# huziqi/NALO-SLAM

Hardware: AMD Instinct MI355X
Metric: keyframes/sec, KITTI-00 dense 8-KF photometric BA; pose RMSE vs ref (higher is better)
Workload: dtype f32; 1 GPU; kitti00_8kf; image=1224x368, levels=4, window_frames=8, active_points=2000, residuals=14000, tracked_frames_per_keyframe=3, multi_gpu=replicas (window too small to shard)

## Files before the change

nalo-slam_amd/csrc/ba_device.h:

```cpp
#pragma once
#include <cstddef>
#include <hip/hip_runtime.h>
#include <cstdint>

namespace nalo {

constexpr int kBlk = 256;
constexpr int kTopVals = 93;
constexpr int kTopStride = 96;
constexpr int kPreStride = 40;
constexpr int kThSmallSlots = 16384;
constexpr int kPreDirectSlots = 32768;
constexpr int kThDblAB = 1024, kThDblC = 256;

enum : uint8_t { RS_STATE_MASK = 3, RS_EXISTS = 4, RS_ACTIVE = 8, RS_LINEARIZED = 16 };
enum : uint8_t { PT_VALID = 1, PT_MARG = 2, PT_HAS_PRIOR = 4, PT_DROP = 8 };
enum : uint8_t { DEC_KEEP = 0, DEC_DROP_NORES = 1, DEC_DROP = 2, DEC_MARGINALIZE = 3 };

struct BADev {
    int W, P, Ppad, nblocks, w, h;
    const float* calib;
    const float4* img[16];
    const float* img_t[16];
    int wt;
    int lin_sub;
    const float* pre;
    float* frameTH;
    const int* blk_host;
    const int* blk_order;
    int xcd_len;
    float4* pt_geo;
    const float4 *pt_col0, *pt_col1, *pt_w0, *pt_w1;
    float* pt_prior;
    uint8_t* pt_flags;
    float4* pt_acc;
    float4* pt_hcd;
    uint8_t* pt_ngood;
    int* pt_numgood; uint32_t* pt_last;
    float* pt_step;
    float* pt_backup;
    const unsigned* gate_p; unsigned* gate_err; unsigned gate_p_want;
    const float* adF;
    float* pt_relbs;
    float* pt_relbs_next;
    uint8_t* rs_state;
    float2* rs_energy;
    float4 *rs_jp0, *rs_jp1;
    float4* rs_pp0; float2* rs_pp1;
    float4* rs_cpt;
    float* en_new;
    double *th_bufAB, *th_bufC;
    unsigned* th_state;
    double* top_partial;
    double* sc_partial;
    int sc_split;
    const int* host_blk;
    const int* sc_grp;
    int sc_bpw, sc_groups;
    int fix_a, fix_b;
    int reset_oob;
    int no_th;
    double* noapply_E;
};

constexpr int kXadArgFrames = 8;
struct XadArg { float v[4 + kXadArgFrames * kXadArgFrames * 8]; };

struct GateBlock { unsigned x_seq, p_seq, err, pad[29]; float x[4 + NALO_MAX_WINDOW * NALO_MAX_WINDOW * 8]; };
static_assert(offsetof(GateBlock, x) == 128, "flags and payload of the gate block on separate cache lines");
constexpr unsigned kGateCancel = 0xFFFFFFFFu;
struct GateArg { const unsigned* flag; unsigned* err; const float* x; unsigned want; };
__device__ __forceinline__ bool gate_wait(const unsigned* flag, unsigned want, unsigned* err) {
    {
        unsigned v0;
        asm volatile("s_load_dword %0, %1, 0x0\n\ts_waitcnt lgkmcnt(0)" : "=s"(v0) : "s"(flag) : "memory");
        if (v0 == want) { __atomic_signal_fence(__ATOMIC_ACQUIRE); return true; }
    }
    for (unsigned spins = 0; spins < (1u << 21); ++spins) {
        const unsigned v = __hip_atomic_load(flag, __ATOMIC_RELAXED, __HIP_MEMORY_SCOPE_SYSTEM);
        if (v == want) { __atomic_signal_fence(__ATOMIC_ACQUIRE); return true; }
        if (v == kGateCancel) return false;
        __builtin_amdgcn_s_sleep(2);
    }
    if (err) __hip_atomic_store(err, 1u, __ATOMIC_RELAXED, __HIP_MEMORY_SCOPE_SYSTEM);
    return false;
}

struct RedExtra {
    const float* th_en; int th_n; float* th_out;
    double* pub; double seq; unsigned* ticket; const float* th_src;
};

struct StitchDev {
    const double* AD;
    const double *M_top, *M_sc;
    double* H;
    unsigned* ticket;
    int W, n1, NPL;
};

struct StitchLayout {
    size_t top, sc, misc, step, th, flag, npub, lo, dev_size, host_size;
    constexpr StitchLayout(int n1, int W)
        : top(0), sc((size_t)n1 * n1), misc(2 * sc), step(misc + 2 * (size_t)W * W), th(step + 3), flag(th + 2), npub(flag),
          lo((npub + 15) & ~(size_t)15), dev_size(lo + kThDblC), host_size(step + 16) {}
};
static_assert(StitchLayout(21, 2).npub - StitchLayout(21, 2).misc == 2 * 2 * 2 + 5 && StitchLayout(21, 2).th - StitchLayout(21, 2).misc == 2 * 2 * 2 + 5 - 2,
              "StitchLayout and ba_reduce_kernel's tail disagree");

struct CarryDev {
    const int* src;
    int trow[16];
    int W_new, Ppad_new, Ppad_old, enter;
    const float4 *o_geo, *o_col0, *o_col1, *o_w0, *o_w1; const float* o_prior; const uint8_t *o_flags, *o_state; const int* o_ng; const uint32_t* o_last;
    float4 *geo, *col0, *col1, *w0, *w1; float* prior; uint8_t *flags, *state; int* ng; uint32_t* last;
    float4 *acc, *hcd; float *step, *backup, *relbs, *relbs2; uint8_t* ngood; float2* energy; float4 *jp0, *jp1, *cpt;
    const float* imm; int immN;
    const int* a_sel; const float* a_idepth; const uint8_t* a_in;
};
void ba_launch_carry(hipStream_t s, const CarryDev& A, int nblocks);

void ba_launch_sc(hipStream_t s, const BADev& B, int T, int shift, float priorScaleMarg, int margOnly);
void ba_launch_linearize(hipStream_t s, const BADev& B, int mode, int fix, hipEvent_t ev_start = nullptr, hipEvent_t ev_stop = nullptr);
void ba_launch_reset_oob(hipStream_t s, const BADev& B);
void ba_launch_restore(hipStream_t s, const BADev& B, const float4* geo, const uint8_t* state, const uint8_t* flags, const float* prior, const float* th);
void ba_launch_reduce(hipStream_t s, const BADev& B, const int* host_blk, int NPL, double* acc13, double* misc, double* G, bool top, bool sc,
                      const float* step_partial, int step_blocks, double* step_out, bool with_th, double* pub, double seq, unsigned* ticket);
void ba_launch_resub_step(hipStream_t s, const BADev& B, float stepfacD, float* partial, const XadArg& karg, bool karg_is_x);
int ba_launch_stitch(hipStream_t s, const StitchDev& D, size_t* lds_allowed, bool top, bool sc, double* mapped, int ntail, double seq);
void ba_launch_resub(hipStream_t s, const BADev& B, const XadArg& karg, bool karg_is_x);
void ba_launch_resub_step_gated(hipStream_t s, const BADev& B, float stepfacD, float* partial, const GateArg& gate);
void ba_launch_pull(hipStream_t s, float* dst, const float* src_mapped, int n);
void ba_launch_step(hipStream_t s, const BADev& B, float stepfacD, float* partial, double* out3);
void ba_launch_step_sums(hipStream_t s, const BADev& B, const float* partial, double* out3);
void ba_launch_publish(hipStream_t s, const double* src, double* dst_mapped, int n, double seq, unsigned* ticket);
void ba_launch_th_install(hipStream_t s, const double* tail2, float* th);
void ba_launch_th_tail(hipStream_t s, const float* th, double* tail2);
void ba_launch_energy_th(hipStream_t s, const BADev& B);
void ba_launch_set_th(hipStream_t s, float* dst, const float* th, int W);
void ba_launch_energy_th_step(hipStream_t s, const BADev& B, int step);
void ba_launch_lenergy(hipStream_t s, const BADev& B, double* partial);
void ba_launch_load_backup(hipStream_t s, const BADev& B);
void ba_launch_swgray(hipStream_t s, const BADev& B, const double* Rt, double* partial);
void ba_launch_set_idepth(hipStream_t s, const BADev& B, int mode, int host_sel, double scale);
void ba_launch_trk_ref_gather(hipStream_t s, const BADev& B, const int* kmap, float* out);
void ba_launch_hist_update(hipStream_t s, const BADev& B, int scrub_only);
void ba_launch_hist_remap(hipStream_t s, const BADev& B, int idx);
void ba_launch_flag_points(hipStream_t s, const BADev& B, unsigned frame_mask, uint8_t* decision, float* idepth_hessian, int* counts, int* counts_next);
void ba_launch_remove_flagged(hipStream_t s, const BADev& B);

}
```

nalo-slam_amd/csrc/host_ba.hip:

```cpp
#include "nalo_internal.h"
#include "ba_device.h"

namespace nalo {

struct HostFrame {
    int slot = 0, frameID = 0;
    SE3 evalPT, PRE_worldToCam, PRE_camToWorld;
    double state[10] = {}, state_zero[10] = {}, state_scaled[10] = {}, step[10] = {}, state_backup[10] = {};
    float ab_exposure = 1.f, frameEnergyTH = 8 * 8 * kPatternNum;
    double prior[8] = {}, delta[8] = {}, delta_prior[8] = {};
    double ns_pose[6][6] = {}, ns_scale[6] = {};
};

struct BAWindow {
    int W = 0, P = 0, Ppad = 0, nblocks = 0, n = 0, n1 = 0, T = 1, NPL = 16;
    double c_value[4] = {}, c_value_zero[4] = {}, c_value_scaled[4] = {}, c_step[4] = {}, c_value_backup[4] = {};
    float c_scaledf[4] = {}, c_scaledi[4] = {};
    std::vector<HostFrame> frames;
    std::vector<double> adHost, adTarget, HM, bM, lastX, Sproj, solve_scratch;
    std::vector<double> ad_key; int ad_key_W = 0;
    std::vector<int> solve_perm;
    std::vector<float> adHostF, adTargetF, adHTdeltaF;
    float cDeltaF[4] = {};
    bool proj_valid = false;
    bool ad_pending = false;
    int resInA = 0, resInL = 0, resInM = 0;
    std::vector<int> d2p, p2d, blk_host_h, host_blk_h;
    std::vector<uint8_t> flags_h;
    BADev dev{};
    DevBuf<float> pre, frameTH, pt_prior, pt_step, pt_backup, pt_relbs, pt_relbs2, en_new, step_partial;
    DevBuf<double> top_partial, sc_partial;
    unsigned long long pub_seq = 0; bool step_pending = false; int last_canbreak = 0; float st_sumA = 0, st_sumB = 0, st_sumT = 0, st_sumR = 0;
    DevBuf<float4> pt_geo, pt_col0, pt_col1, pt_w0, pt_w1, pt_acc, pt_hcd, rs_jp0, rs_jp1, rs_cpt;
    DevBuf<float2> rs_energy, rs_pp1;
    DevBuf<float4> rs_pp0;
    DevBuf<uint8_t> pt_flags, pt_ngood, rs_state;
    DevBuf<int> blk_host, host_blk, blk_order, sc_grp;
    DevBuf<unsigned> th_hist;
    bool step_fused = false, step_sums_deferred = false;
    bool th_pending = false;
    DevBuf<double> acc13, G, AD, stitched;
    StitchLayout lay = StitchLayout(0, 0);
    size_t stitch_lds_allowed = 48 * 1024;
    DevBuf<unsigned> st_ticket;
    StitchDev sd{};
    HostBuf<double> ad_host;
    Event ev_ad;
    HostBuf<double> stitched_host;
    HostBuf<float> up_host;
    HostBuf<float> pre_map[4]; long pre_pos = 0, pre_synced = 0;
    bool have_lin = false, have_sc = false, stitched_top = false, stitched_sc = false, points_set = false, res_set = false;
    bool pt_acc_on_read = false;
    int sc_shift = -1;
    DevBuf<float4> snap_geo; DevBuf<uint8_t> snap_state, snap_flags; DevBuf<float> snap_prior;
    std::vector<HostFrame> snap_frames; std::vector<double> snap_HM, snap_bM; std::vector<uint8_t> snap_flags_h; bool have_snap = false;
    double snap_calib[4] = {}, snap_calib_scaled[4] = {}; float snap_scaledf[4] = {}, snap_scaledi[4] = {};
    HostBuf<GateBlock> gate_h; unsigned gate_x_seq = 0, gate_p_seq = 0;
    bool want_prelaunch = false, resub_pre = false, lin_pre = false;
    nalo_allreduce_fn hook = nullptr;
    void* hook_user = nullptr;
    bool hook_stream_ordered = false;
    nalo_allreduce_fn hook_side = nullptr; void* hook_side_user = nullptr;
    DevBuf<double> th_buf;
    Event ev_lin, ev_th; bool th_side_inflight = false;
    bool th_lo_pending = false;
    bool never_break = false;
    DevBuf<double> small_sum;
    DevBuf<double> noapply_E; std::vector<double> noapply_h;
    int opt_iterations = 0, opt_rejected = 0;
    bool prior_next = false;
    bool prior_carry = false;
    bool lin_fixed = false;
    std::vector<int> ref_kmap_h; DevBuf<int> ref_kmap; bool ref_kmap_ok = false;
    DevBuf<float> ref_in;
    DevBuf<int> pt_numgood, snap_numgood; DevBuf<uint32_t> pt_last, snap_last;
    bool hist_set = false, snap_hist = false;
    DevBuf<uint8_t> flag_dec; DevBuf<float> flag_H; DevBuf<int> flag_counts; int flag_buf = 0;
    bool flagged = false;
    DevBuf<float4> pt_geo2, pt_col0_2, pt_col1_2, pt_w0_2, pt_w1_2; DevBuf<float> pt_prior2; DevBuf<uint8_t> pt_flags2, rs_state2; DevBuf<int> pt_numgood2; DevBuf<uint32_t> pt_last2;
    std::vector<unsigned long long> key_h;
    std::vector<int> row_of;
    bool carry_ok = false;
    unsigned frames_epoch = 0;
    HostBuf<int> carry_host; DevBuf<int> carry_src; Event ev_carry;
    std::vector<int> carry_map_h; int carry_stats[4] = {}; bool carried = false;
};

void ba_destroy(nalo_ctx* c) {
    delete c->ba;
    c->ba = nullptr;
}

static void calib_set_value(BAWindow& w, const double v[4]) {
    for (int i = 0; i < 4; ++i) w.c_value[i] = v[i];
    w.c_value_scaled[0] = kScaleF * v[0]; w.c_value_scaled[1] = kScaleF * v[1]; w.c_value_scaled[2] = kScaleC * v[2]; w.c_value_scaled[3] = kScaleC * v[3];
    for (int i = 0; i < 4; ++i) w.c_scaledf[i] = (float)w.c_value_scaled[i];
    w.c_scaledi[0] = 1.0f / w.c_scaledf[0]; w.c_scaledi[1] = 1.0f / w.c_scaledf[1];
    w.c_scaledi[2] = -w.c_scaledf[2] / w.c_scaledf[0]; w.c_scaledi[3] = -w.c_scaledf[3] / w.c_scaledf[1];
}
static void frame_set_state(HostFrame& f, const double st[10]) {
    std::memcpy(f.state, st, sizeof(f.state));
    for (int i = 0; i < 3; ++i) f.state_scaled[i] = kScaleXiTrans * st[i];
    for (int i = 3; i < 6; ++i) f.state_scaled[i] = kScaleXiRot * st[i];
    f.state_scaled[6] = kScaleA * st[6]; f.state_scaled[7] = kScaleB * st[7]; f.state_scaled[8] = kScaleA * st[8]; f.state_scaled[9] = kScaleB * st[9];
    f.PRE_worldToCam = se3_exp(f.state_scaled) * f.evalPT;
    f.PRE_camToWorld = f.PRE_worldToCam.inverse();
}
static void frame_set_state_zero(HostFrame& f, const double sz[10]) {
    std::memcpy(f.state_zero, sz, sizeof(f.state_zero));
    const SE3 inv = f.evalPT.inverse();
    for (int i = 0; i < 6; ++i) {
        double eps[6] = {0, 0, 0, 0, 0, 0}, lp[6], lm[6];
        eps[i] = 1e-3; const SE3 P = (f.evalPT * se3_exp(eps)) * inv;
        eps[i] = -1e-3; const SE3 M = (f.evalPT * se3_exp(eps)) * inv;
        se3_log(P, lp); se3_log(M, lm);
        for (int r = 0; r < 6; ++r) f.ns_pose[i][r] = (lp[r] - lm[r]) / (2e-3);
    }
    SE3 P = f.evalPT, M = f.evalPT;
    for (int i = 0; i < 3; ++i) { P.m[i * 4 + 3] *= 1.00001; M.m[i * 4 + 3] /= 1.00001; }
    double lp[6], lm[6];
    se3_log(P * inv, lp); se3_log(M * inv, lm);
    for (int r = 0; r < 6; ++r) f.ns_scale[r] = (lp[r] - lm[r]) / (2e-3);
}
static void frame_take_data(const nalo_settings& set, HostFrame& f) {
    double p[8] = {0, 0, 0, 0, 0, 0, 0, 0};
    if (f.frameID == 0) { for (int i = 0; i < 3; ++i) p[i] = kInitialTransPrior; for (int i = 3; i < 6; ++i) p[i] = kInitialRotPrior; p[6] = kInitialAffPrior; p[7] = kInitialAffPrior; }
    else { p[6] = set.affineOptModeA < 0 ? kInitialAffPrior : set.affineOptModeA; p[7] = set.affineOptModeB < 0 ? kInitialAffPrior : set.affineOptModeB; }
    for (int i = 0; i < 8; ++i) { f.prior[i] = p[i]; f.delta[i] = f.state[i] - f.state_zero[i]; f.delta_prior[i] = f.state[i]; }
}

static int upload_adjoints(nalo_ctx* c);
static int set_adjoints(nalo_ctx* c, bool defer = false) {
    BAWindow& w = *c->ba;
    HostTimer ht(c, "ba.set_adjoints");
    const int W = w.W, n1 = w.n1;
    constexpr int KEY = 15;
    std::vector<uint8_t> dirty(W, 1);
    if (w.ad_key_W == W && w.ad_key.size() == (size_t)W * KEY && w.adHost.size() == (size_t)W * W * 64) {
        for (int f = 0; f < W; ++f) {
            double k[KEY]; std::memcpy(k, w.frames[f].evalPT.m, 12 * sizeof(double)); k[12] = w.frames[f].ab_exposure; k[13] = w.frames[f].state_zero[6]; k[14] = w.frames[f].state_zero[7];
// ... 216 lines not shown
        hipStream_t st = on_side ? c->side : c->stream;
        nalo_allreduce_fn fn = (on_side && w.hook_side) ? w.hook_side : w.hook;
        void* user = (on_side && w.hook_side) ? w.hook_side_user : w.hook_user;
        if (on_side) NALO_HIP(c, hipStreamWaitEvent(c->side, lin_done, 0));
        for (int lvl = 0; lvl < 2; ++lvl) {
            ba_launch_energy_th_step(st, w.dev, lvl);
            if (!w.hook_stream_ordered) NALO_HIP(c, hipStreamSynchronize(st));
            { int rh = call_hook(c, fn, user, w.th_buf.p + lvl * kThDblAB, kThDblAB); if (rh) return rh; }
        }
        ba_launch_energy_th_step(st, w.dev, 2);
        if (on_side) { NALO_HIP(c, hipEventRecord(w.ev_th, c->side)); w.th_side_inflight = true; }
        w.th_lo_pending = true;
    } else if (mode == 0) w.th_pending = true;
    if (fix != 2) { w.have_lin = true; w.have_sc = false; w.stitched_top = false; w.stitched_sc = false; }
    NALO_HIP(c, hipGetLastError());
    w.lin_fixed = mode == 0 && fix == 1;
    return NALO_OK;
}
static int linearize_noapply(nalo_ctx* c, double* E) {
    BAWindow& w = *c->ba;
    const size_t n = (size_t)w.nblocks * w.dev.lin_sub * w.W;
    NALO_HIP(c, w.noapply_E.reserve(n));
    w.dev.noapply_E = w.noapply_E.p;
    NALO_HIP(c, hipMemsetAsync(w.noapply_E.p, 0, n * sizeof(double), c->stream));
    int rc = linearize_async(c, 0, 2); if (rc) return rc;
    w.noapply_h.resize(n);
    NALO_HIP(c, hipMemcpyAsync(w.noapply_h.data(), w.noapply_E.p, n * sizeof(double), hipMemcpyDeviceToHost, c->stream));
    NALO_HIP(c, hipStreamSynchronize(c->stream));
    double s = 0; for (double v : w.noapply_h) s += v;
    { int rs = sum_over_ranks(c, &s, 1); if (rs) return rs; }
    *E = s;
    return NALO_OK;
}
static int calc_l_energy(nalo_ctx* c, double* E) {
    BAWindow& w = *c->ba;
    double e = 0;
    for (const auto& f : w.frames) for (int i = 0; i < 8; ++i) e += f.delta_prior[i] * f.prior[i] * f.delta_prior[i];
    { float ec = 0; for (int i = 0; i < 4; ++i) ec += (w.cDeltaF[i] * (float)kInitialCalibHessian) * w.cDeltaF[i]; e += ec; }
    const int nb = (w.Ppad + 255) / 256;
    NALO_HIP(c, w.noapply_E.reserve((size_t)std::max<size_t>(nb, (size_t)w.nblocks * w.dev.lin_sub * w.W)));
    ba_launch_lenergy(c->stream, w.dev, w.noapply_E.p);
    std::vector<double> part(nb);
    NALO_HIP(c, hipMemcpyAsync(part.data(), w.noapply_E.p, nb * sizeof(double), hipMemcpyDeviceToHost, c->stream));
    NALO_HIP(c, hipStreamSynchronize(c->stream));
    double ep = 0; for (double v : part) ep += v;
    { int rs = sum_over_ranks(c, &ep, 1); if (rs) return rs; }
    *E = e + (double)(float)ep;
    return NALO_OK;
}
static double calc_m_energy(const BAWindow& w) {
    const int n = w.n;
    std::vector<double> d(n);
    for (int i = 0; i < 4; ++i) d[i] = (double)w.cDeltaF[i];
    for (int h = 0; h < w.W; ++h) for (int i = 0; i < 8; ++i) d[4 + 8 * h + i] = w.frames[h].delta[i];
    double E = 0;
    for (int i = 0; i < n; ++i) { double s = 0; for (int j = 0; j < n; ++j) s += w.HM[(size_t)i * n + j] * d[j]; E += d[i] * (2 * w.bM[i] + s); }
    return E;
}
static int load_state_backup(nalo_ctx* c) {
    BAWindow& w = *c->ba;
    calib_set_value(w, w.c_value_backup);
    for (auto& f : w.frames) frame_set_state(f, f.state_backup);
    ba_launch_load_backup(c->stream, w.dev);
    NALO_HIP(c, hipGetLastError());
    return set_precalc(c);
}
static int sc_async(nalo_ctx* c, int shift, float margScale, int margOnly) {
    BAWindow& w = *c->ba;
    ProfScope ps(c, "ba_sc");
    ba_launch_sc(c->stream, w.dev, w.T, shift, margScale, margOnly);
    w.have_sc = true; w.sc_shift = shift; w.stitched_sc = false;
    NALO_HIP(c, hipGetLastError());
    return NALO_OK;
}
static bool prelaunch_eligible(const nalo_ctx* c, const BAWindow& w) {
    return !w.hook && c->set.forceAcceptStep && w.points_set && w.Ppad <= kPreDirectSlots && w.W <= 8;
}
static int prelaunch_iteration(nalo_ctx* c) {
    BAWindow& w = *c->ba;
    if (!w.gate_h.p) {
        NALO_HIP(c, w.gate_h.reserve(1, hipHostMallocMapped | hipHostMallocCoherent));
        std::memset(w.gate_h.p, 0, sizeof(GateBlock));
    }
    GateBlock* const gh = w.gate_h.p; GateBlock* const gd = w.gate_h.dev;
    if (w.pre_pos + 1 - 4 > w.pre_synced || !w.pre_map[0].dev) return NALO_OK;
    if (gh->x_seq == kGateCancel) __atomic_store_n(&gh->x_seq, 0u, __ATOMIC_RELEASE);
    if (gh->p_seq == kGateCancel) __atomic_store_n(&gh->p_seq, 0u, __ATOMIC_RELEASE);
    if (++w.gate_x_seq == kGateCancel) w.gate_x_seq = 1;
    if (++w.gate_p_seq == kGateCancel) w.gate_p_seq = 1;
    {
        ProfScope ps(c, "ba_resub");
        NALO_HIP(c, w.step_partial.reserve((size_t)(w.Ppad / 256 + 1) * 4));
        const GateArg g{&gd->x_seq, &gd->err, gd->x, w.gate_x_seq};
        ba_launch_resub_step_gated(c->stream, w.dev, 1.f, w.step_partial.p, g);
    }
    w.resub_pre = true;
    {
        BADev D = w.dev;
        const size_t nfl = (size_t)w.W * w.W * kPreStride;
        D.pre = w.pre_map[(w.pre_pos + 1) & 3].dev; D.calib = D.pre + nfl;
        D.gate_p = &gd->p_seq; D.gate_err = &gd->err; D.gate_p_want = w.gate_p_seq;
        ProfScope ps(c, "ba_linearize", true);
        ba_launch_linearize(c->stream, D, 0, 0, ps.a, ps.b);
    }
    w.lin_pre = true;
    NALO_HIP(c, hipGetLastError());
    return NALO_OK;
}
static void prelaunch_cancel(nalo_ctx* c) {
    BAWindow& w = *c->ba;
    if (!(w.resub_pre || w.lin_pre) || !w.gate_h.p) return;
    __atomic_store_n(&w.gate_h.p->x_seq, kGateCancel, __ATOMIC_RELEASE); __atomic_store_n(&w.gate_h.p->p_seq, kGateCancel, __ATOMIC_RELEASE);
    (void)hipStreamSynchronize(c->stream);
    w.resub_pre = w.lin_pre = false; w.want_prelaunch = false;
    w.have_lin = false; w.have_sc = false;
}

static int stitch_and_fetch(nalo_ctx* c, bool want_top, bool want_sc, bool th_to_host = false, bool misc_only = false) {
    BAWindow& w = *c->ba;
    if (w.ad_pending && !misc_only) { int ra = upload_adjoints(c); if (ra) return ra; }
    const int NPL = w.NPL, W = w.W;
    const StitchLayout& L = w.lay;
    bool did = false;
    const int ntail = (int)(L.npub - L.misc);
    const double seq = (double)(w.pub_seq + 1);
    double* const dmap = w.stitched_host.dev;
    const bool top = want_top && !w.stitched_top, sc = want_sc && !w.stitched_sc;
    const bool sc_was_summed = w.stitched_sc;
    const bool fuse_lo = w.hook && w.th_lo_pending && (top || misc_only);
    bool th_after_publish = false;
    {
        const bool small_th = !w.hook && w.th_pending && th_to_host && w.dev.Ppad <= kThSmallSlots && (top || sc);
        const bool pub_in_reduce = misc_only && !w.hook && (top || sc) && (small_th || !w.th_pending);
        if ((top || sc) && (th_to_host || w.hook) && !fuse_lo && !pub_in_reduce) {
            if (!small_th) { int rc = flush_th(c); if (rc) return rc; }
            if (!small_th) ba_launch_th_tail(c->stream, w.frameTH.p + (W - 1), w.stitched.p + L.th);
        }
        ProfScope ps(c, "ba_reduce");
        if (top || sc) {
            ba_launch_reduce(c->stream, w.dev, w.host_blk.p, NPL, w.acc13.p, w.stitched.p + L.misc, w.G.p, top, sc,
                             w.step_sums_deferred ? w.step_partial.p : nullptr, (w.Ppad + 255) / 256, w.stitched.p + L.step, small_th,
                             pub_in_reduce ? dmap + L.misc : nullptr, seq, w.st_ticket.p + 2);
            if (small_th) w.th_pending = false;
            w.step_sums_deferred = false;
            if (misc_only) { if (!w.hook && !pub_in_reduce) ba_launch_publish(c->stream, w.stitched.p + L.misc, dmap + L.misc, ntail, seq, w.st_ticket.p + 1); }
            else {
                if (small_th && th_to_host) ba_launch_th_tail(c->stream, w.frameTH.p + (W - 1), w.stitched.p + L.th);
                if (ba_launch_stitch(c->stream, w.sd, &w.stitch_lds_allowed, top, sc, w.hook ? nullptr : dmap, ntail, seq)) return fail(c, NALO_ERR_HIP, "ba_stitch_kernel: LDS size rejected");
                if (top) w.stitched_top = true;
                if (sc) w.stitched_sc = true;
            }
            did = true;
        }
    }
    NALO_HIP(c, hipGetLastError());
    if (did) {
        ++w.pub_seq;
        if (w.hook) {
            const size_t off = misc_only ? L.misc : 0;
            const size_t tail_end = fuse_lo ? L.lo + kThDblC : L.npub;
            size_t ra[2], rb[2]; int nr = 0;
            if (misc_only) { ra[nr] = L.misc; rb[nr++] = tail_end; }
            else if (top && (sc || !sc_was_summed)) { ra[nr] = L.top; rb[nr++] = tail_end; }
            else if (top) { ra[nr] = L.top; rb[nr++] = L.sc; ra[nr] = L.misc; rb[nr++] = tail_end; }
            else { ra[nr] = L.sc; rb[nr++] = L.misc; }
            if (fuse_lo) {
                if (w.th_side_inflight) { NALO_HIP(c, hipStreamWaitEvent(c->stream, w.ev_th, 0)); w.th_side_inflight = false; }
                w.th_lo_pending = false;
            }
            if (!w.hook_stream_ordered) NALO_HIP(c, hipStreamSynchronize(c->stream));
            for (int i = 0; i < nr; ++i) { int rh = call_hook(c, w.hook, w.hook_user, w.stitched.p + ra[i], (int)(rb[i] - ra[i])); if (rh) return rh; }
            if (fuse_lo) {
                if (th_to_host) {
                    ba_launch_energy_th_step(c->stream, w.dev, 3);
                    ba_launch_th_tail(c->stream, w.frameTH.p + (W - 1), w.stitched.p + L.th);
                } else th_after_publish = true;
            } else if (top || misc_only) ba_launch_th_install(c->stream, w.stitched.p + L.th, w.frameTH.p + (W - 1));
            ba_launch_publish(c->stream, w.stitched.p + off, dmap + off, (int)(L.npub - off), seq, w.st_ticket.p + 1);
            if (th_after_publish) ba_launch_energy_th_step(c->stream, w.dev, 3);
            NALO_HIP(c, hipGetLastError());
        }
        { int rc = flush_th(c); if (rc) return rc; }
        if (w.want_prelaunch) { w.want_prelaunch = false; int rc = prelaunch_iteration(c); if (rc) return rc; }
        if (!poll_flag(c, &w.stitched_host.p[L.flag], seq)) return NALO_ERR_HIP;
// ... 1402 lines not shown
```

nalo-slam_amd/csrc/kernels_ba.hip:

```cpp
#include "nalo_internal.h"
#include "ba_device.h"
#include "reduce.h"

namespace nalo {


__global__ __launch_bounds__(256) void ba_reset_oob_kernel(uint8_t* __restrict__ rs_state, float2* __restrict__ rs_energy, size_t n) {
    const size_t i = (size_t)blockIdx.x * blockDim.x + threadIdx.x;
    if (i >= n) return;
    const uint8_t st = rs_state[i];
    if ((st & RS_EXISTS) && !(st & RS_LINEARIZED)) { rs_state[i] = (uint8_t)(st & ~RS_STATE_MASK); rs_energy[i] = make_float2(0.f, 0.f); }
}

struct ScPoint { float4 pa; float4 hc; int ngood; };
__device__ __forceinline__ void sc_point_finish(const BADev& B, int d, ScPoint& P, float prior, float idepth, float idepth_zero, int margOnly, float priorScaleMarg, int shiftPriorToZero) {
    B.pt_hcd[d] = P.hc; B.pt_ngood[d] = (uint8_t)P.ngood;
    if (P.ngood == 0) { P.pa.z = 0.f; P.pa.w = 0.f; }
    else {
        if (margOnly) { prior *= priorScaleMarg; B.pt_prior[d] = prior; }
        float Hs = P.pa.x + prior;
        if (Hs < 1e-10f) Hs = 1e-10f;
        P.pa.z = (float)(1.0 / (double)Hs);
        P.pa.w = P.pa.y;
        if (shiftPriorToZero) P.pa.w += prior * (idepth - idepth_zero);
// ... 559 lines not shown
                if (c < 4) { for (int q = 0; q < nb; ++q) s += U[q * 104 + r * 13 + c]; }
                else if (c == n) { for (int q = 0; q < nb; ++q) s += U[q * 104 + r * 13 + 12]; }
                else {
                    const int j = (c - 4) >> 3, cp = (c - 4) & 7;
                    if (j == a) {
                        for (int q = 0; q < nb; ++q)
#pragma unroll
                            for (int k = 0; k < 8; ++k) s += U[q * 104 + r * 13 + 4 + k] * As[q * kAdMat + cp * kAdRow + k];
                    } else {
                        const int jj = j < a ? j : j - 1, q1 = jj, q2 = W - 1 + jj;
#pragma unroll
                        for (int k = 0; k < 8; ++k) s += U[q1 * 104 + r * 13 + 4 + k] * Ao[q1 * kAdMat + cp * kAdRow + k];
#pragma unroll
                        for (int k = 0; k < 8; ++k) s += U[q2 * 104 + r * 13 + 4 + k] * Ao[q2 * kAdMat + cp * kAdRow + k];
                    }
                }
                put(4 + 8 * a + r, c, s);
                if (c < 4 || c == n) put(c, 4 + 8 * a + r, s);
            }
        } else if (sys == 0) {
            for (int e = tid; e < W * W * 25; e += NT) {
                const int bin = e / 25, o = e - bin * 25, ri = o / 5, ci = o - ri * 5;
                lds[e] = (bin % W != bin / W) ? D.M_top[(size_t)bin * 169 + (ri < 4 ? ri : 12) * 13 + (ci < 4 ? ci : 12)] : 0.0;
            }
            __syncthreads();
            for (int e = tid; e < 25; e += NT) {
                const int ri = e / 5, ci = e - ri * 5;
                double s = 0;
                for (int bin = 0; bin < W * W; ++bin) s += lds[bin * 25 + e];
                put(ri < 4 ? ri : n, ci < 4 ? ci : n, s);
            }
        } else if (g < W) {
            if (ad_in_lds) { if (D.W == 8) stitch_sc_rows<true, 8>(D, lds, g, r0, 8 / kScSplit, put); else stitch_sc_rows<true, 0>(D, lds, g, r0, 8 / kScSplit, put); }
            else stitch_sc_rows<false, 0>(D, lds, g, r0, 8 / kScSplit, put);
        } else {
            const int cb = 8 * (W - 1);
            for (int e = tid; e < W * 25; e += NT) {
                const int i = e / 25, o = e - i * 25, ri = o / 5, ci = o - ri * 5;
                lds[e] = D.M_sc[(size_t)i * NPL * NPL + (size_t)(cb + ri) * NPL + cb + ci];
            }
            __syncthreads();
            for (int e = tid; e < 25; e += NT) {
                const int ri = e / 5, ci = e - ri * 5;
                double s = 0;
                for (int i = 0; i < W; ++i) s += lds[i * 25 + e];
                put(ri < 4 ? ri : n, ci < 4 ? ci : n, s);
            }
        }
    }
    if (!mapped) return;
    __builtin_amdgcn_fence(__ATOMIC_RELEASE, "workgroup");
    __syncthreads();
    if (tid == 0) is_last = __hip_atomic_fetch_add(D.ticket, 1u, __ATOMIC_RELAXED, __HIP_MEMORY_SCOPE_AGENT) == gridDim.x - 1u;
    __syncthreads();
    if (!is_last) return;
    const size_t t0 = (size_t)2 * n1 * n1;
    for (int i = tid; i < ntail; i += NT) __hip_atomic_store(&mapped[t0 + i], D.H[t0 + i], __ATOMIC_RELAXED, __HIP_MEMORY_SCOPE_SYSTEM);
    __builtin_amdgcn_fence(__ATOMIC_RELEASE, "workgroup");
    __syncthreads();
    if (tid == 0) {
        __hip_atomic_store(D.ticket, 0u, __ATOMIC_RELAXED, __HIP_MEMORY_SCOPE_AGENT);
        __hip_atomic_store(&mapped[t0 + ntail], seq, __ATOMIC_RELEASE, __HIP_MEMORY_SCOPE_SYSTEM);
    }
}
int ba_launch_stitch(hipStream_t s, const StitchDev& D, size_t* lds_allowed, bool top, bool sc, double* mapped, int ntail, double seq) {
    const int mask = (top ? 1 : 0) | (sc ? 2 : 0);
    const size_t lds_top = (size_t)2 * (D.W - 1) * (169 + 2 * kAdMat + 104) * 8, lds_ad = (size_t)2 * D.W * D.W * kAdMat * 8;
    size_t lds_sc = (size_t)D.W * 8 * D.NPL * 8;
    const size_t lds_p1 = ((size_t)D.NPL * D.NPL + (size_t)D.W * 8 * D.NPL + (size_t)2 * D.W * 64) * 8;
    const size_t lds_stage = lds_p1 > lds_ad ? lds_p1 : lds_ad;
    const int ad_in_lds = lds_sc + lds_stage <= 156 * 1024;
    if (ad_in_lds) lds_sc += lds_stage;
    size_t lds = lds_top > lds_sc ? lds_top : lds_sc;
    if (lds < (size_t)D.W * D.W * 25 * 8) lds = (size_t)D.W * D.W * 25 * 8;
    if (lds > *lds_allowed) {
        if (hipFuncSetAttribute((const void*)ba_stitch_kernel, hipFuncAttributeMaxDynamicSharedMemorySize, (int)lds) != hipSuccess) return 1;
        *lds_allowed = lds;
    }
    ba_stitch_kernel<<<(kScSplit + kTopSplit) * D.W + 2, 1024, lds, s>>>(D, mask, ad_in_lds, mapped, ntail, seq);
    return 0;
}

template <bool STEP, int XMODE>
__global__ __launch_bounds__(256) void ba_resub_kernel(BADev B, XadArg X, GateArg G, float stepfacD, float* __restrict__ partial) {
    __shared__ float smem[64 * 4];
    __shared__ float xrow[XMODE >= 2 ? NALO_MAX_WINDOW * 8 + 4 : 1];
    constexpr bool KARG = XMODE == 1;
    static_assert(XMODE >= 1 && XMODE <= 3, "x or xAd arrive as kernel arguments, or (3) through the gate block");
    const float* xc = XMODE == 3 ? xrow + NALO_MAX_WINDOW * 8 : X.v;
    const float* xAd = X.v + 4;
    if constexpr (XMODE == 3) {
        __shared__ int gate_ok;
        const int tid = threadIdx.x, W = B.W;
        if (tid == 0) gate_ok = gate_wait(G.flag, G.want, G.err) ? 1 : 0;
        __syncthreads();
        if (!gate_ok) return;
        const int hb = B.blk_host[blockIdx.x];
        if (tid < W * 8) xrow[tid] = G.x[4 + (size_t)hb * W * 8 + tid];
        else if (tid >= 252) xrow[NALO_MAX_WINDOW * 8 + tid - 252] = G.x[tid - 252];
        __syncthreads();
    }
    if constexpr (XMODE == 2) {
        const int hb = B.blk_host[blockIdx.x], W = B.W, tid = threadIdx.x;
        if (tid < W * 8) {
            const int t = tid >> 3, j = tid & 7;
            const float* AH = B.adF + (size_t)(hb + W * t) * 64 + j;
            const float* AT = B.adF + (size_t)W * W * 64 + (size_t)(hb + W * t) * 64 + j;
            float s1 = 0.f, s2 = 0.f;
#pragma unroll
            for (int i = 0; i < 8; ++i) { s1 = __fadd_rn(s1, __fmul_rn(X.v[4 + 8 * hb + i], AH[i * 8])); s2 = __fadd_rn(s2, __fmul_rn(X.v[4 + 8 * t + i], AT[i * 8])); }
            xrow[tid] = __fadd_rn(s1, s2);
        }
        __syncthreads();
    }
    const int d = blockIdx.x * blockDim.x + threadIdx.x;
    float v[3] = {0.f, 0.f, 0.f};
    if (d < B.Ppad && (B.pt_flags[d] & PT_VALID)) {
        const int h = __builtin_amdgcn_readfirstlane(B.blk_host[blockIdx.x]), W = B.W;
        float stp = 0.f;
        if (B.pt_ngood[d] != 0) {
            const float4 pa = B.pt_acc[d], hc = B.pt_hcd[d];
            float bsum = pa.w;
            bsum -= xc[0] * hc.x + xc[1] * hc.y + xc[2] * hc.z + xc[3] * hc.w;
            if constexpr (KARG || XMODE == 3) {
                for (int t0 = 0; t0 < W; t0 += 8) {
                    uint8_t rs[8]; float4 j0[8], j1[8];
#pragma unroll
                    for (int i = 0; i < 8; ++i) {
                        rs[i] = 0; j0[i] = make_float4(0.f, 0.f, 0.f, 0.f); j1[i] = j0[i];
                        if (t0 + i < W) {
                            const size_t si = (size_t)(t0 + i) * B.Ppad + d;
                            rs[i] = B.rs_state[si]; j0[i] = B.rs_jp0[si]; j1[i] = B.rs_jp1[si];
                        }
                    }
#pragma unroll
                    for (int i = 0; i < 8; ++i) {
                        const int t = t0 + i;
                        const float* xa = XMODE == 3 ? xrow + min(t, W - 1) * 8 : xAd + (size_t)(h * W + min(t, W - 1)) * 8;
                        const float term = xa[0] * j0[i].x + xa[1] * j0[i].y + xa[2] * j0[i].z + xa[3] * j0[i].w + xa[4] * j1[i].x + xa[5] * j1[i].y + xa[6] * j1[i].z + xa[7] * j1[i].w;
                        if (t < W && t != h && (rs[i] & RS_ACTIVE)) bsum -= term;
                    }
                }
            } else {
                for (int t0 = 0; t0 < W; t0 += 8) {
                    uint8_t rs[8]; float4 j0[8], j1[8];
#pragma unroll
                    for (int i = 0; i < 8; ++i) { const int t = t0 + i; rs[i] = (t < W && t != h) ? B.rs_state[(size_t)t * B.Ppad + d] : 0; }
#pragma unroll
                    for (int i = 0; i < 8; ++i) {
                        const int t = t0 + i;
                        const bool on = t < W && (rs[i] & RS_ACTIVE);
                        const size_t si = (size_t)(on ? t : 0) * B.Ppad + d;
                        j0[i] = B.rs_jp0[si]; j1[i] = B.rs_jp1[si];
                        if (!on) rs[i] = 0;
                    }
#pragma unroll
                    for (int i = 0; i < 8; ++i) {
                        const int t = t0 + i;
                        const float* xa = XMODE >= 2 ? xrow + min(t, W - 1) * 8 : xAd + (size_t)(h * W + min(t, W - 1)) * 8;
                        const float term = xa[0] * j0[i].x + xa[1] * j0[i].y + xa[2] * j0[i].z + xa[3] * j0[i].w + xa[4] * j1[i].x + xa[5] * j1[i].y + xa[6] * j1[i].z + xa[7] * j1[i].w;
                        if (rs[i] & RS_ACTIVE) bsum -= term;
                    }
                }
            }
            stp = -bsum * pa.z;
        }
        B.pt_step[d] = stp;
        if (STEP) {
            float4 geo = B.pt_geo[d];
            const float idb = geo.z;
            B.pt_backup[d] = idb;
            geo.z = idb + stepfacD * stp; geo.w = geo.z;
            B.pt_geo[d] = geo;
            v[0] = stp * stp; v[1] = fabsf(idb); v[2] = 1.f;
        }
    }
    if (STEP) block_reduce_cols<3, 256>(v, smem, partial + (size_t)blockIdx.x * 4);
}
__global__ __launch_bounds__(256) void ba_step_kernel(BADev B, float stepfacD, float* __restrict__ partial ) {
    __shared__ float smem[64 * 4];
    const int d = blockIdx.x * blockDim.x + threadIdx.x;
    float v[3] = {0.f, 0.f, 0.f};
    if (d < B.Ppad && (B.pt_flags[d] & PT_VALID)) {
        float4 geo = B.pt_geo[d];
        const float idb = geo.z, stp = B.pt_step[d];
        B.pt_backup[d] = idb;
        geo.z = idb + stepfacD * stp; geo.w = geo.z;
        B.pt_geo[d] = geo;
        v[0] = stp * stp; v[1] = fabsf(idb); v[2] = 1.f;
    }
    block_reduce_cols<3, 256>(v, smem, partial + (size_t)blockIdx.x * 4);
}
__global__ __launch_bounds__(1024) void ba_sum_partials_kernel(const float* __restrict__ partial, int nblocks, int stride, int nvals, double* __restrict__ out) {
    __shared__ double part[1024];
    const int L = nvals <= 4 ? 4 : 64, NG = 1024 / L;
    const int j = threadIdx.x % L, g = threadIdx.x / L;
    double s = 0;
    if (j < nvals) for (int b = g; b < nblocks; b += NG) s += (double)partial[(size_t)b * stride + j];
    part[g * L + j] = s;
    __syncthreads();
    if (g == 0 && j < nvals) { double t = 0; for (int k = 0; k < NG; ++k) t += part[k * L + j]; out[j] = t; }
}
__global__ __launch_bounds__(256) void ba_publish_kernel(const double* __restrict__ src, double* __restrict__ dst, int n, double seq, unsigned* __restrict__ ticket) {
    __shared__ int is_last;
    for (int i = blockIdx.x * blockDim.x + threadIdx.x; i < n; i += gridDim.x * blockDim.x) __hip_atomic_store(&dst[i], src[i], __ATOMIC_RELAXED, __HIP_MEMORY_SCOPE_SYSTEM);
    __builtin_amdgcn_fence(__ATOMIC_RELEASE, "workgroup");
    __syncthreads();
    if (threadIdx.x == 0) is_last = __hip_atomic_fetch_add(ticket, 1u, __ATOMIC_RELAXED, __HIP_MEMORY_SCOPE_AGENT) == gridDim.x - 1u;
    __syncthreads();
    if (is_last && threadIdx.x == 0) {
        __hip_atomic_store(ticket, 0u, __ATOMIC_RELAXED, __HIP_MEMORY_SCOPE_AGENT);
        __hip_atomic_store(&dst[n], seq, __ATOMIC_RELEASE, __HIP_MEMORY_SCOPE_SYSTEM);
    }
}
__global__ void ba_th_install_kernel(const double* __restrict__ tail2, float* __restrict__ th) { if (tail2[1] > 1.5) th[0] = (float)(tail2[0] / tail2[1]); }
void ba_launch_th_install(hipStream_t s, const double* tail2, float* th) { ba_th_install_kernel<<<1, 1, 0, s>>>(tail2, th); }
__global__ void ba_th_tail_kernel(const float* __restrict__ th, double* __restrict__ tail2) { tail2[0] = (double)th[0]; tail2[1] = 1.0; }
void ba_launch_th_tail(hipStream_t s, const float* th, double* tail2) { ba_th_tail_kernel<<<1, 1, 0, s>>>(th, tail2); }
void ba_launch_publish(hipStream_t s, const double* src, double* dst_mapped, int n, double seq, unsigned* ticket) {
    const int nb = n > 32768 ? 32 : (n + 1023) / 1024;
    ba_publish_kernel<<<nb < 1 ? 1 : nb, 256, 0, s>>>(src, dst_mapped, n, seq, ticket);
}
__global__ __launch_bounds__(1024) void ba_pull_kernel(float4* __restrict__ dst, const float4* __restrict__ src_mapped, int n4) {
    for (int i = threadIdx.x; i < n4; i += 1024) dst[i] = src_mapped[i];
}
void ba_launch_pull(hipStream_t s, float* dst, const float* src_mapped, int n) { ba_pull_kernel<<<1, 1024, 0, s>>>((float4*)dst, (const float4*)src_mapped, (n + 3) / 4); }
void ba_launch_resub(hipStream_t s, const BADev& B, const XadArg& karg, bool karg_is_x) {
    const GateArg none{};
    if (karg_is_x) ba_resub_kernel<false, 2><<<(B.Ppad + 255) / 256, 256, 0, s>>>(B, karg, none, 0.f, nullptr);
    else ba_resub_kernel<false, 1><<<(B.Ppad + 255) / 256, 256, 0, s>>>(B, karg, none, 0.f, nullptr);
}
void ba_launch_resub_step(hipStream_t s, const BADev& B, float stepfacD, float* partial, const XadArg& karg, bool karg_is_x) {
    const GateArg none{};
    if (karg_is_x) ba_resub_kernel<true, 2><<<(B.Ppad + 255) / 256, 256, 0, s>>>(B, karg, none, stepfacD, partial);
    else ba_resub_kernel<true, 1><<<(B.Ppad + 255) / 256, 256, 0, s>>>(B, karg, none, stepfacD, partial);
}
void ba_launch_resub_step_gated(hipStream_t s, const BADev& B, float stepfacD, float* partial, const GateArg& gate) {
    static const XadArg none{};
    ba_resub_kernel<true, 3><<<(B.Ppad + 255) / 256, 256, 0, s>>>(B, none, gate, stepfacD, partial);
}
void ba_launch_step_sums(hipStream_t s, const BADev& B, const float* partial, double* out3) { ba_sum_partials_kernel<<<1, 1024, 0, s>>>(partial, (B.Ppad + 255) / 256, 4, 3, out3); }
void ba_launch_step(hipStream_t s, const BADev& B, float stepfacD, float* partial, double* out3) {
    const int nb = (B.Ppad + 255) / 256;
    ba_step_kernel<<<nb, 256, 0, s>>>(B, stepfacD, partial);
    ba_sum_partials_kernel<<<1, 1024, 0, s>>>(partial, nb, 4, 3, out3);
}

constexpr int kThBinsAB = 2048, kThBinsC = 512;
constexpr double kThPack = 67108864.0;
template <int NBINS>
__device__ __forceinline__ void th_search(const double* __restrict__ buf, bool first, unsigned k_in, unsigned* s, unsigned& total, unsigned& k, unsigned& bin, unsigned& before) {
    constexpr int NB = NBINS / 256;
    const int tid = threadIdx.x, lane = tid & 63, wave = tid >> 6;
    unsigned cnt[NB], sum = 0;
#pragma unroll
    for (int j = 0; j < NB / 2; ++j) {
        const unsigned long long v = (unsigned long long)(buf[tid * (NB / 2) + j] + 0.5);
        cnt[2 * j] = (unsigned)(v & 0x3FFFFFFull); cnt[2 * j + 1] = (unsigned)(v >> 26);
        sum += cnt[2 * j] + cnt[2 * j + 1];
    }
    unsigned incl = sum;
#pragma unroll
    for (int o = 1; o < 64; o <<= 1) { const unsigned t = __shfl_up(incl, o); if (lane >= o) incl += t; }
    if (lane == 63) s[wave] = incl;
    if (tid == 0) { s[4] = (unsigned)(NBINS - 1); s[5] = 0u; }
    __syncthreads();
    unsigned wpre = 0;
    total = s[0] + s[1] + s[2] + s[3];
    for (int i = 0; i < wave; ++i) wpre += s[i];
    k = first ? (unsigned)(int)(kFrameEnergyTHN * (float)total) : k_in;
    const unsigned excl = wpre + incl - sum;
    if (excl <= k && k < excl + sum) {
        unsigned run = excl; int b = 0; bool found = false;
#pragma unroll
        for (int j = 0; j < NB; ++j) { if (!found && k < run + cnt[j]) { b = j; found = true; } if (!found) run += cnt[j]; }
        s[4] = (unsigned)(tid * NB + b); s[5] = run;
    }
    __syncthreads();
    bin = s[4]; before = s[5];
}
template <int LEVEL>
__global__ __launch_bounds__(256) void ba_th_fill_kernel(const float* __restrict__ en, int n, const double* __restrict__ prev, unsigned* __restrict__ state, double* __restrict__ out) {
    constexpr int NB = LEVEL == 2 ? kThBinsC : kThBinsAB;
    __shared__ unsigned hist[NB];
    __shared__ unsigned s[8];
    const int tid = threadIdx.x;
    unsigned prefix = 0;
    if (LEVEL == 1) {
        unsigned total, k, bin, before;
        th_search<kThBinsAB>(prev, true, 0u, s, total, k, bin, before);
        if (blockIdx.x == 0 && tid == 0) { state[0] = total; state[3] = total == 0 ? 1u : 0u; state[1] = k - before; state[2] = bin; }
        prefix = bin;
    }
    if (LEVEL == 2) {
        unsigned total, k, bin, before;
        const unsigned binA = state[2];
        th_search<kThBinsAB>(prev, false, state[1], s, total, k, bin, before);
        if (blockIdx.x == 0 && tid == 0) { state[4] = k - before; state[5] = bin; }
        prefix = (binA << 11) | bin;
    }
    for (int b = tid; b < NB; b += 256) hist[b] = 0u;
    __syncthreads();
    for (int i = blockIdx.x * 256 + tid; i < n; i += gridDim.x * 256) {
        const float f = en[i];
        if (!(f >= 0.f)) continue;
        const unsigned u = __float_as_uint(f);
        if (LEVEL == 0) atomicAdd(&hist[u >> 20], 1u);
        if (LEVEL == 1) { if ((u >> 20) == prefix) atomicAdd(&hist[(u >> 9) & 2047u], 1u); }
        if (LEVEL == 2) { if ((u >> 9) == prefix) atomicAdd(&hist[u & 511u], 1u); }
    }
    __syncthreads();
    for (int b = tid; b < NB / 2; b += 256) {
        const unsigned c0 = hist[2 * b], c1 = hist[2 * b + 1];
        if (c0 | c1) unsafeAtomicAdd(&out[b], (double)c0 + (double)c1 * kThPack);
    }
}
__global__ __launch_bounds__(256) void ba_th_final_kernel(double* __restrict__ bufC, const unsigned* __restrict__ state, double* __restrict__ bufAB, float* __restrict__ frameTH_new) {
    __shared__ unsigned s[8];
    const int tid = threadIdx.x;
    unsigned total, k, bin, before;
    th_search<kThBinsC>(bufC, false, state[4], s, total, k, bin, before);
    if (tid == 0) {
// ... 215 lines not shown
```

Baseline: 961.9 keyframes/s.

## Prefetch per-point state before gate wait and pull pre-buffer into device memory

The gated resub kernel now loads each thread's point flags, accumulators, geometry and per-frame Jacobians before spinning on the host gate, so those loads overlap the wait. It also launches one extra workgroup that waits on the second gate and copies the mapped host pre-buffer into device memory, then publishes a device-side ready flag. Linearize then reads the pre data and the gate from device memory instead of host-mapped memory. This costs extra registers per thread in the resub kernel and adds a copy plus an acquire fence.

Result: no change. 964.7 keyframes/s (median of 4 runs) (+0.3%).

```diff
diff --git a/nalo-slam_amd/csrc/ba_device.h b/nalo-slam_amd/csrc/ba_device.h
--- a/nalo-slam_amd/csrc/ba_device.h
+++ b/nalo-slam_amd/csrc/ba_device.h
@@ -70,15 +70,17 @@
 static_assert(offsetof(GateBlock, x) == 128, "flags and payload of the gate block on separate cache lines");
 constexpr unsigned kGateCancel = 0xFFFFFFFFu;
 struct GateArg { const unsigned* flag; unsigned* err; const float* x; unsigned want; };
+struct PullArg { const unsigned* flag = nullptr; unsigned* err = nullptr; unsigned want = 0; int wg = -1; const float4* src = nullptr; float4* dst = nullptr; int n4 = 0; unsigned* ready = nullptr; };
+template <bool ACQUIRE = false>
 __device__ __forceinline__ bool gate_wait(const unsigned* flag, unsigned want, unsigned* err) {
     {
         unsigned v0;
         asm volatile("s_load_dword %0, %1, 0x0\n\ts_waitcnt lgkmcnt(0)" : "=s"(v0) : "s"(flag) : "memory");
-        if (v0 == want) { __atomic_signal_fence(__ATOMIC_ACQUIRE); return true; }
+        if (v0 == want) { if constexpr (ACQUIRE) __builtin_amdgcn_fence(__ATOMIC_ACQUIRE, ""); else __atomic_signal_fence(__ATOMIC_ACQUIRE); return true; }
     }
     for (unsigned spins = 0; spins < (1u << 21); ++spins) {
         const unsigned v = __hip_atomic_load(flag, __ATOMIC_RELAXED, __HIP_MEMORY_SCOPE_SYSTEM);
-        if (v == want) { __atomic_signal_fence(__ATOMIC_ACQUIRE); return true; }
+        if (v == want) { if constexpr (ACQUIRE) __builtin_amdgcn_fence(__ATOMIC_ACQUIRE, ""); else __atomic_signal_fence(__ATOMIC_ACQUIRE); return true; }
         if (v == kGateCancel) return false;
         __builtin_amdgcn_s_sleep(2);
     }
@@ -129,7 +131,7 @@
 void ba_launch_resub_step(hipStream_t s, const BADev& B, float stepfacD, float* partial, const XadArg& karg, bool karg_is_x);
 int ba_launch_stitch(hipStream_t s, const StitchDev& D, size_t* lds_allowed, bool top, bool sc, double* mapped, int ntail, double seq);
 void ba_launch_resub(hipStream_t s, const BADev& B, const XadArg& karg, bool karg_is_x);
-void ba_launch_resub_step_gated(hipStream_t s, const BADev& B, float stepfacD, float* partial, const GateArg& gate);
+void ba_launch_resub_step_gated(hipStream_t s, const BADev& B, float stepfacD, float* partial, const GateArg& gate, const PullArg& pull);
 void ba_launch_pull(hipStream_t s, float* dst, const float* src_mapped, int n);
 void ba_launch_step(hipStream_t s, const BADev& B, float stepfacD, float* partial, double* out3);
 void ba_launch_step_sums(hipStream_t s, const BADev& B, const float* partial, double* out3);
diff --git a/nalo-slam_amd/csrc/host_ba.hip b/nalo-slam_amd/csrc/host_ba.hip
--- a/nalo-slam_amd/csrc/host_ba.hip
+++ b/nalo-slam_amd/csrc/host_ba.hip
@@ -56,6 +56,7 @@
     std::vector<HostFrame> snap_frames; std::vector<double> snap_HM, snap_bM; std::vector<uint8_t> snap_flags_h; bool have_snap = false;
     double snap_calib[4] = {}, snap_calib_scaled[4] = {}; float snap_scaledf[4] = {}, snap_scaledi[4] = {};
     HostBuf<GateBlock> gate_h; unsigned gate_x_seq = 0, gate_p_seq = 0;
+    DevBuf<unsigned> gate_d;
     bool want_prelaunch = false, resub_pre = false, lin_pre = false;
     nalo_allreduce_fn hook = nullptr;
     void* hook_user = nullptr;
@@ -438,24 +439,33 @@
         NALO_HIP(c, w.gate_h.reserve(1, hipHostMallocMapped | hipHostMallocCoherent));
         std::memset(w.gate_h.p, 0, sizeof(GateBlock));
     }
+    if (!w.gate_d.p) {
+        NALO_HIP(c, w.gate_d.reserve(32));
+        NALO_HIP(c, hipMemsetAsync(w.gate_d.p, 0, 32 * sizeof(unsigned), c->stream));
+    }
     GateBlock* const gh = w.gate_h.p; GateBlock* const gd = w.gate_h.dev;
     if (w.pre_pos + 1 - 4 > w.pre_synced || !w.pre_map[0].dev) return NALO_OK;
     if (gh->x_seq == kGateCancel) __atomic_store_n(&gh->x_seq, 0u, __ATOMIC_RELEASE);
     if (gh->p_seq == kGateCancel) __atomic_store_n(&gh->p_seq, 0u, __ATOMIC_RELEASE);
     if (++w.gate_x_seq == kGateCancel) w.gate_x_seq = 1;
     if (++w.gate_p_seq == kGateCancel) w.gate_p_seq = 1;
+    const size_t nfl = (size_t)w.W * w.W * kPreStride;
+    NALO_HIP(c, w.pre.reserve(nfl + 32));
     {
         ProfScope ps(c, "ba_resub");
         NALO_HIP(c, w.step_partial.reserve((size_t)(w.Ppad / 256 + 1) * 4));
         const GateArg g{&gd->x_seq, &gd->err, gd->x, w.gate_x_seq};
-        ba_launch_resub_step_gated(c->stream, w.dev, 1.f, w.step_partial.p, g);
+        PullArg pl;
+        pl.flag = &gd->p_seq; pl.err = &gd->err; pl.want = w.gate_p_seq; pl.wg = (w.dev.Ppad + 255) / 256;
+        pl.src = reinterpret_cast<const float4*>(w.pre_map[(w.pre_pos + 1) & 3].dev); pl.dst = reinterpret_cast<float4*>(w.pre.p);
+        pl.n4 = (int)((nfl + 16 + 3) / 4); pl.ready = w.gate_d.p;
+        ba_launch_resub_step_gated(c->stream, w.dev, 1.f, w.step_partial.p, g, pl);
     }
     w.resub_pre = true;
     {
         BADev D = w.dev;
-        const size_t nfl = (size_t)w.W * w.W * kPreStride;
-        D.pre = w.pre_map[(w.pre_pos + 1) & 3].dev; D.calib = D.pre + nfl;
-        D.gate_p = &gd->p_seq; D.gate_err = &gd->err; D.gate_p_want = w.gate_p_seq;
+        D.pre = w.pre.p; D.calib = D.pre + nfl;
+        D.gate_p = w.gate_d.p; D.gate_err = &gd->err; D.gate_p_want = w.gate_p_seq;
         ProfScope ps(c, "ba_linearize", true);
         ba_launch_linearize(c->stream, D, 0, 0, ps.a, ps.b);
     }
diff --git a/nalo-slam_amd/csrc/kernels_ba.hip b/nalo-slam_amd/csrc/kernels_ba.hip
--- a/nalo-slam_amd/csrc/kernels_ba.hip
+++ b/nalo-slam_amd/csrc/kernels_ba.hip
@@ -665,20 +665,45 @@
 }
 
 template <bool STEP, int XMODE>
-__global__ __launch_bounds__(256) void ba_resub_kernel(BADev B, XadArg X, GateArg G, float stepfacD, float* __restrict__ partial) {
+__global__ __launch_bounds__(256) void ba_resub_kernel(BADev B, XadArg X, GateArg G, PullArg P, float stepfacD, float* __restrict__ partial) {
     __shared__ float smem[64 * 4];
     __shared__ float xrow[XMODE >= 2 ? NALO_MAX_WINDOW * 8 + 4 : 1];
     constexpr bool KARG = XMODE == 1;
     static_assert(XMODE >= 1 && XMODE <= 3, "x or xAd arrive as kernel arguments, or (3) through the gate block");
     const float* xc = XMODE == 3 ? xrow + NALO_MAX_WINDOW * 8 : X.v;
     const float* xAd = X.v + 4;
+    uint8_t g_fl = 0, g_ng = 0, g_rs[8]; float4 g_pa, g_hc, g_geo, g_j0[8], g_j1[8]; int g_hb = 0;
     if constexpr (XMODE == 3) {
         __shared__ int gate_ok;
         const int tid = threadIdx.x, W = B.W;
-        if (tid == 0) gate_ok = gate_wait(G.flag, G.want, G.err) ? 1 : 0;
+        if ((int)blockIdx.x == P.wg) {
+            if (tid == 0) gate_ok = gate_wait<true>(P.flag, P.want, P.err) ? 1 : 0;
+            __syncthreads();
+            if (gate_ok) {
+                float4 r[3];
+#pragma unroll
+                for (int k = 0; k < 3; ++k) r[k] = P.src[min(tid + k * 256, P.n4 - 1)];
+#pragma unroll
+                for (int k = 0; k < 3; ++k) if (tid + k * 256 < P.n4) P.dst[tid + k * 256] = r[k];
+                for (int i = tid + 768; i < P.n4; i += 256) P.dst[i] = P.src[i];
+            }
+            if (tid == 0) *P.ready = gate_ok ? P.want : kGateCancel;
+            return;
+        }
+        const int hb = g_hb = B.blk_host[blockIdx.x];
+        const int d = min((int)blockIdx.x * 256 + tid, B.Ppad - 1);
+        g_fl = B.pt_flags[d]; g_ng = B.pt_ngood[d]; g_pa = B.pt_acc[d]; g_hc = B.pt_hcd[d]; g_geo = B.pt_geo[d];
+#pragma unroll
+        for (int i = 0; i < 8; ++i) {
+            g_rs[i] = 0; g_j0[i] = make_float4(0.f, 0.f, 0.f, 0.f); g_j1[i] = g_j0[i];
+            if (i < W) {
+                const size_t si = (size_t)i * B.Ppad + d;
+                g_rs[i] = B.rs_state[si]; g_j0[i] = B.rs_jp0[si]; g_j1[i] = B.rs_jp1[si];
+            }
+        }
+        if (tid == 0) gate_ok = gate_wait<true>(G.flag, G.want, G.err) ? 1 : 0;
         __syncthreads();
         if (!gate_ok) return;
-        const int hb = B.blk_host[blockIdx.x];
         if (tid < W * 8) xrow[tid] = G.x[4 + (size_t)hb * W * 8 + tid];
         else if (tid >= 252) xrow[NALO_MAX_WINDOW * 8 + tid - 252] = G.x[tid - 252];
         __syncthreads();
@@ -698,11 +723,11 @@
     }
     const int d = blockIdx.x * blockDim.x + threadIdx.x;
     float v[3] = {0.f, 0.f, 0.f};
-    if (d < B.Ppad && (B.pt_flags[d] & PT_VALID)) {
-        const int h = __builtin_amdgcn_readfirstlane(B.blk_host[blockIdx.x]), W = B.W;
+    if (d < B.Ppad && ((XMODE == 3 ? g_fl : B.pt_flags[d]) & PT_VALID)) {
+        const int h = __builtin_amdgcn_readfirstlane(XMODE == 3 ? g_hb : B.blk_host[blockIdx.x]), W = B.W;
         float stp = 0.f;
-        if (B.pt_ngood[d] != 0) {
-            const float4 pa = B.pt_acc[d], hc = B.pt_hcd[d];
+        if ((XMODE == 3 ? g_ng : B.pt_ngood[d]) != 0) {
+            const float4 pa = XMODE == 3 ? g_pa : B.pt_acc[d], hc = XMODE == 3 ? g_hc : B.pt_hcd[d];
             float bsum = pa.w;
             bsum -= xc[0] * hc.x + xc[1] * hc.y + xc[2] * hc.z + xc[3] * hc.w;
             if constexpr (KARG || XMODE == 3) {
@@ -711,7 +736,8 @@
 #pragma unroll
                     for (int i = 0; i < 8; ++i) {
                         rs[i] = 0; j0[i] = make_float4(0.f, 0.f, 0.f, 0.f); j1[i] = j0[i];
-                        if (t0 + i < W) {
+                        if constexpr (XMODE == 3) { rs[i] = g_rs[i]; j0[i] = g_j0[i]; j1[i] = g_j1[i]; }
+                        else if (t0 + i < W) {
                             const size_t si = (size_t)(t0 + i) * B.Ppad + d;
                             rs[i] = B.rs_state[si]; j0[i] = B.rs_jp0[si]; j1[i] = B.rs_jp1[si];
                         }
@@ -750,7 +776,7 @@
         }
         B.pt_step[d] = stp;
         if (STEP) {
-            float4 geo = B.pt_geo[d];
+            float4 geo = XMODE == 3 ? g_geo : B.pt_geo[d];
             const float idb = geo.z;
             B.pt_backup[d] = idb;
             geo.z = idb + stepfacD * stp; geo.w = geo.z;
@@ -809,18 +835,19 @@
 }
 void ba_launch_pull(hipStream_t s, float* dst, const float* src_mapped, int n) { ba_pull_kernel<<<1, 1024, 0, s>>>((float4*)dst, (const float4*)src_mapped, (n + 3) / 4); }
 void ba_launch_resub(hipStream_t s, const BADev& B, const XadArg& karg, bool karg_is_x) {
-    const GateArg none{};
-    if (karg_is_x) ba_resub_kernel<false, 2><<<(B.Ppad + 255) / 256, 256, 0, s>>>(B, karg, none, 0.f, nullptr);
-    else ba_resub_kernel<false, 1><<<(B.Ppad + 255) / 256, 256, 0, s>>>(B, karg, none, 0.f, nullptr);
+    const GateArg none{}; const PullArg nop{};
+    if (karg_is_x) ba_resub_kernel<false, 2><<<(B.Ppad + 255) / 256, 256, 0, s>>>(B, karg, none, nop, 0.f, nullptr);
+    else ba_resub_kernel<false, 1><<<(B.Ppad + 255) / 256, 256, 0, s>>>(B, karg, none, nop, 0.f, nullptr);
 }
 void ba_launch_resub_step(hipStream_t s, const BADev& B, float stepfacD, float* partial, const XadArg& karg, bool karg_is_x) {
-    const GateArg none{};
-    if (karg_is_x) ba_resub_kernel<true, 2><<<(B.Ppad + 255) / 256, 256, 0, s>>>(B, karg, none, stepfacD, partial);
-    else ba_resub_kernel<true, 1><<<(B.Ppad + 255) / 256, 256, 0, s>>>(B, karg, none, stepfacD, partial);
-}
-void ba_launch_resub_step_gated(hipStream_t s, const BADev& B, float stepfacD, float* partial, const GateArg& gate) {
+    const GateArg none{}; const PullArg nop{};
+    if (karg_is_x) ba_resub_kernel<true, 2><<<(B.Ppad + 255) / 256, 256, 0, s>>>(B, karg, none, nop, stepfacD, partial);
+    else ba_resub_kernel<true, 1><<<(B.Ppad + 255) / 256, 256, 0, s>>>(B, karg, none, nop, stepfacD, partial);
+}
+void ba_launch_resub_step_gated(hipStream_t s, const BADev& B, float stepfacD, float* partial, const GateArg& gate, const PullArg& pull) {
     static const XadArg none{};
-    ba_resub_kernel<true, 3><<<(B.Ppad + 255) / 256, 256, 0, s>>>(B, none, gate, stepfacD, partial);
+    const int nb = (B.Ppad + 255) / 256;
+    ba_resub_kernel<true, 3><<<nb + (pull.wg == nb ? 1 : 0), 256, 0, s>>>(B, none, gate, pull, stepfacD, partial);
 }
 void ba_launch_step_sums(hipStream_t s, const BADev& B, const float* partial, double* out3) { ba_sum_partials_kernel<<<1, 1024, 0, s>>>(partial, (B.Ppad + 255) / 256, 4, 3, out3); }
 void ba_launch_step(hipStream_t s, const BADev& B, float stepfacD, float* partial, double* out3) {
```
